# Axionis47/GAT-Recommendation

Hardware: AMD Instinct MI355X
Metric: training sessions/sec + Recall@10 parity, 82k-node graph, 1/2/4/8 MI355X (higher is better)
Workload: dtype fp32

## Files before the change

### gat-recommendation_amd/csrc/gtr_opt.hip

```cpp

#include <hipcub/hipcub.hpp>
#include <rocprim/device/device_radix_sort.hpp>

#include <cstdarg>
#include <cstdio>

#include "gtr_rows.cuh"
#include <string.h>

#include "gtr_wgrad.cuh"

namespace gtr {

static thread_local char g_err[512] = "";

void set_error(const char* fmt, ...) {
  va_list ap;
  va_start(ap, fmt);
  vsnprintf(g_err, sizeof(g_err), fmt, ap);
  va_end(ap);
}

}

// ... 693 lines not shown
      s_acc[tid] = acc;
      __syncthreads();
      if (tid == 0) {
        float t = 0.0f;
        for (int q = 0; q < GTR_BLOCK; ++q) t += s_acc[q];
        a.tl.loss_out[0] = t;
        if (a.tl.loss_acc) a.tl.loss_acc[0] += (double)t;
      }
    } else if (blk == 0 && a.tl.loss_acc && tid == 0) {
      a.tl.loss_acc[0] += (double)a.tl.loss_out[0];
    }
  }
}

struct WgradRowsK {
  WgradK w;
  gtr_batch bt;
  gtr_tail tl;
  gtr_adam opt;
  int T, nb_wg;
};

template <int D>
__global__ __launch_bounds__(GTR_TAIL_BLOCK) void k_wgrad_rows(WgradRowsK a) {
  const int blk = blockIdx.x, tid = threadIdx.x;
  if (blk < a.nb_wg) {
    if (tid >= GTR_BLOCK) return;
    wgrad_block(a.w, blk);
    return;
  }
  __shared__ AdamStep s_st;
  __shared__ int32_t s_t;
  __shared__ int s_ready;
  if (tid == 0) s_ready = 0;
  __syncthreads();
  if (tid >= GTR_BLOCK) {
    if (tid == GTR_BLOCK) {
      const int64_t t = *a.opt.step_dev + a.opt.step_offset;
      s_st.init(a.opt, t);
      s_t = (int32_t)t;
      __hip_atomic_store(&s_ready, 1, __ATOMIC_RELEASE, __HIP_MEMORY_SCOPE_WORKGROUP);
    }
    return;
  }
  auto wait = [&]() {
    while (__hip_atomic_load(&s_ready, __ATOMIC_ACQUIRE, __HIP_MEMORY_SCOPE_WORKGROUP) == 0)
      __builtin_amdgcn_s_sleep(1);
  };
  rows_body<D>((blk - a.nb_wg) * GTR_BLOCK + tid, a.bt, a.T, a.tl.skeys, a.tl.svals, a.tl.dx0, a.tl.se,
               a.tl.coef_tgt, a.tl.coef_neg, a.tl.table, a.tl.table_m, a.tl.table_v, nullptr, s_st,
               a.tl.lazy_consts ? a.tl.stamp : nullptr, s_t, wait);
}

template <int D>
__global__ __launch_bounds__(GTR_BLOCK) void k_scatter_rows(gtr_batch bt, int mode, const float* src,
                                                            const float* coef_tgt, const float* coef_neg,
                                                            float* dense) {
  constexpr int VPL = D >= 64 ? D / 64 : 1;
  const int lane = threadIdx.x & 63, wave = threadIdx.x >> 6;
  const int r = blockIdx.x * GTR_WAVES + wave;
  const int d0 = lane * VPL;
  if (d0 >= D) return;
  const int N = bt.hdr[0], B = bt.hdr[1];
  int key;
  const float* s;
  float c;
  if (mode == 0) {
    if (r >= N) return;
    key = bt.node_item[r];
    s = src + (size_t)r * D;
    c = 1.0f;
  } else {
    if (r >= B * (1 + bt.n_neg)) return;
    if (r < B) {
      key = bt.target[r];
      s = src + (size_t)r * D;
      c = coef_tgt[r];
    } else {
      const int q = r - B;
      key = bt.negatives[q];
      s = src + (size_t)(q / bt.n_neg) * D;
      c = coef_neg[q];
    }
  }
  if (key <= 0) return;
#pragma unroll
  for (int q = 0; q < VPL; ++q) atomicAdd(dense + (size_t)key * D + d0 + q, c * s[d0 + q]);
}

__global__ void k_step_end(int64_t* step_dev, uint32_t* rng_ctr, const float* loss_part, int nparts,
                           float* loss_out) {
  __shared__ float s_acc[64];
  const int tid = threadIdx.x;
  float acc = 0.0f;
  if (loss_part)
    for (int q = tid; q < nparts; q += 64) acc += loss_part[(size_t)q * 2] + loss_part[(size_t)q * 2 + 1];
  s_acc[tid] = acc;
  __syncthreads();
  if (tid == 0) {
    if (loss_part && loss_out) {
      float t = 0.0f;
      for (int q = 0; q < 64; ++q) t += s_acc[q];
      loss_out[0] = t;
    }
    if (step_dev) *step_dev += 1;
    if (rng_ctr) *rng_ctr += 1;
// ... 975 lines not shown
  k.bt = *bt;
  k.tl = t;
  k.opt = *opt;
  k.T = num_items;
  k.D = D;
  k.P = n_chunks;
  k.stride = slab_stride;
  k.cnt = tile_cnt;
  const char* wm = getenv("GTR_WGRAD");
  bool mfma = (bt->n_cap + n_chunks - 1) / n_chunks >= GTR_WGRAD_MFMA_ROWS;
  if (wm && !strcmp(wm, "mfma")) mfma = true;
  if (wm && !strcmp(wm, "valu")) mfma = false;
  if (slab_stride % 4) mfma = false;
  for (int l = 0; l < cfg->num_layers; ++l)
    if (reinterpret_cast<uintptr_t>(layer_slab[l]) % 16) mfma = false;
  int nj = 0, wblocks = 0;
  const int rc = build_wjobs(cfg, bt, layers, t.dx0, pe_tab, layer_slab, pe_slab, layer_flat, pe_flat, n_chunks, 0,
                             cfg->num_layers, k.jobs, nj, wblocks, mfma);
  if (rc) return rc;
  int tiles = 0;
  for (int i = 0; i < nj; ++i) {
    k.jobs[i].tile0 = tiles;
    tiles += k.jobs[i].nt;
    if (k.jobs[i].fW < 0 && k.jobs[i].fB < 0) { set_error("gtr_step_tail_wgrad: a job without flat offsets"); return GTR_E_ARG; }
  }
  if (tiles > tile_cnt_len) {
    set_error("gtr_step_tail_wgrad: %d tile counters needed, %d given", tiles, tile_cnt_len);
    return GTR_E_ARG;
  }
  k.njobs = nj;
  k.nb_wg = wblocks;
  k.nb_rows = (int)(((int64_t)m_cap * (D / 4) + GTR_BLOCK - 1) / GTR_BLOCK);
  int64_t tot = 0;
  for (int i = 0; i < nseg; ++i) {
    k.segs[i] = segs[i];
    tot += segs[i].len;
  }
  k.nseg = nseg;
  k.small_total = (int)tot;
  k.nb_small = (int)((tot + GTR_BLOCK - 1) / GTR_BLOCK);
  if (k.nb_small == 0 && (t.loss_part || t.loss_acc)) k.nb_small = 1;
  const int grid = k.nb_wg + k.nb_rows + k.nb_small;
  hipStream_t s = (hipStream_t)stream;
  switch (D) {
    case 32: hipLaunchKernelGGL(k_step_tail_wgrad<32>, dim3(grid), dim3(GTR_BLOCK), 0, s, k); break;
    case 64: hipLaunchKernelGGL(k_step_tail_wgrad<64>, dim3(grid), dim3(GTR_BLOCK), 0, s, k); break;
    case 128: hipLaunchKernelGGL(k_step_tail_wgrad<128>, dim3(grid), dim3(GTR_BLOCK), 0, s, k); break;
    default: hipLaunchKernelGGL(k_step_tail_wgrad<256>, dim3(grid), dim3(GTR_BLOCK), 0, s, k); break;
  }
  GTR_HIP_CHECK_LAUNCH();
  return GTR_OK;
}

static bool dp_layout_ok(const gtr_dp_layout* l, int dim) {
  return l && l->world >= 1 && l->m_cap > 0 && l->flat_total >= 0 && l->loss_off >= l->flat_total &&
         l->keys_off > l->loss_off && l->rows_off >= l->keys_off + l->m_cap && (l->rows_off & 3) == 0 &&
         l->words >= l->rows_off + (int64_t)l->m_cap * dim && (l->words & 3) == 0;
}

int gtr_dp_pack(const gtr_batch* bt, int num_items, int dim, const gtr_tail* tail, const gtr_segment* segs, int nseg,
                const gtr_dp_layout* lay, float* pack, gtr_stream_t stream) {
  if (!bt || !tail || !pack || !dim_ok(dim) || !dp_layout_ok(lay, dim) || nseg < 0 || nseg > GTR_SMALL_MAX_SEG ||
      lay->m_cap != bt->n_cap + bt->b_cap * (1 + bt->n_neg) || !tail->skeys || !tail->svals || !tail->dx0 ||
      !tail->se || !tail->coef_tgt || !tail->coef_neg || (!tail->loss_part && !tail->loss_out)) {
    set_error("gtr_dp_pack: bad arguments");
    return GTR_E_ARG;
  }
  DpPackK k{};
  k.bt = *bt;
  k.tl = *tail;
  k.lay = *lay;
  k.pack = pack;
  k.T = num_items;
  hipStream_t s = (hipStream_t)stream;
  k.windowed = lay->m_cap > GTR_BEGIN_MCAP ? 1 : 0;
  if (k.windowed) {
    if (!tail->carry) { set_error("gtr_dp_pack: large batch (m_cap > %d) needs the carry scratch", GTR_BEGIN_MCAP); return GTR_E_ARG; }
    const int nwin = (lay->m_cap + TW - 1) / TW;
    k.nb_rows = nwin;
    if (nwin > 1) {
      switch (dim) {
        case 32: hipLaunchKernelGGL(k_tail_carry<32>, dim3(carry_blocks(lay->m_cap)), dim3(GTR_BLOCK), 0, s, *bt, num_items, *tail); break;
        case 64: hipLaunchKernelGGL(k_tail_carry<64>, dim3(carry_blocks(lay->m_cap)), dim3(GTR_BLOCK), 0, s, *bt, num_items, *tail); break;
        case 128: hipLaunchKernelGGL(k_tail_carry<128>, dim3(carry_blocks(lay->m_cap)), dim3(GTR_BLOCK), 0, s, *bt, num_items, *tail); break;
        default: hipLaunchKernelGGL(k_tail_carry<256>, dim3(carry_blocks(lay->m_cap)), dim3(GTR_BLOCK), 0, s, *bt, num_items, *tail); break;
      }
      GTR_HIP_CHECK_LAUNCH();
    }
  } else {
    k.nb_rows = (int)(((int64_t)lay->m_cap * (dim / 4) + GTR_BLOCK - 1) / GTR_BLOCK);
  }
  k.nb_small = (int)((lay->flat_total + GTR_BLOCK - 1) / GTR_BLOCK);
  if (k.nb_small == 0) k.nb_small = 1;
  k.nseg = nseg;
  for (int i = 0; i < nseg; ++i) k.segs[i] = segs[i];
  const int grid = k.nb_rows + k.nb_small;
  switch (dim) {
    case 32: hipLaunchKernelGGL(k_dp_pack<32>, dim3(grid), dim3(GTR_BLOCK), 0, s, k); break;
    case 64: hipLaunchKernelGGL(k_dp_pack<64>, dim3(grid), dim3(GTR_BLOCK), 0, s, k); break;
    case 128: hipLaunchKernelGGL(k_dp_pack<128>, dim3(grid), dim3(GTR_BLOCK), 0, s, k); break;
    default: hipLaunchKernelGGL(k_dp_pack<256>, dim3(grid), dim3(GTR_BLOCK), 0, s, k); break;
  }
  GTR_HIP_CHECK_LAUNCH();
  return GTR_OK;
}

// ... 55 lines not shown
```

### gat-recommendation_amd/etpgt/backend/_lib.py

```python

from __future__ import annotations

import ctypes as C
import os

_HERE = os.path.dirname(os.path.abspath(__file__))
PKG_ROOT = os.path.dirname(os.path.dirname(_HERE))
LIB_PATH = os.environ.get("GTR_LIB", os.path.join(PKG_ROOT, "build", "libgtr_hip.so"))

P = C.c_void_p
i32 = C.c_int32
i64 = C.c_int64
f32 = C.c_float
u32 = C.c_uint32


class GtrBatch(C.Structure):
    _fields_ = [
        ("hdr", P), ("node_item", P), ("node_ptr", P), ("in_ptr", P), ("in_src", P),
        ("out_ptr", P), ("out_edge", P), ("out_dst", P), ("target", P), ("negatives", P),
        ("node_pe", P), ("grp_row", P), ("grp_edge", P),
        ("n_cap", i32), ("b_cap", i32), ("e_cap", i32), ("n_neg", i32),
    ]

# ... 94 lines not shown
        ("flat_total", i64), ("loss_off", i64), ("keys_off", i64), ("rows_off", i64), ("words", i64),
        ("m_cap", i32), ("world", i32),
    ]


class GtrShard(C.Structure):
    _fields_ = [
        ("num_items", i32), ("world", i32), ("rank", i32), ("cap", i32), ("local_rows", i32), ("dim", i32),
        ("table", P), ("m", P), ("v", P), ("stamp", P), ("consts", P), ("consts_cap", i32), ("cap_s", i32),
        ("status", P), ("opt", GtrAdam), ("node_mark", P), ("grad_stride", i64), ("small_stride", i64),
        ("pack_parts", i32), ("pad1", i32),
    ]


GTR_LOSS = {"none": 0, "bpr": 1, "listwise": 2, "sampled_softmax": 2, "dual": 3}
RO_FWD, RO_LOSS, RO_BWD = 1, 2, 4
SMALL_MAX_SEG = 48

_SIGS = {
    "gtr_version": (C.c_int, []),
    "gtr_abi_version": (C.c_int, []),
    "gtr_source_hash": (C.c_char_p, []),
    "gtr_last_error": (C.c_char_p, []),
    "gtr_device_check": (C.c_int, [C.c_int]),
    "gtr_conv_fwd": (C.c_int, [P, P, P, P, C.c_int, P]),
    "gtr_readout_loss": (C.c_int, [P, P, P, P, P, P]),
    "gtr_conv_bwd": (C.c_int, [P, P, P, C.c_int, P, P]),
    "gtr_qkvs_fwd": (C.c_int, [P, P, P, P, C.c_int, P]),
    "gtr_attn_fwd": (C.c_int, [P, P, P, C.c_int, P]),
    "gtr_attn_bwd": (C.c_int, [P, P, P, C.c_int, P]),
    "gtr_qkvs_bwd": (C.c_int, [P, P, P, C.c_int, P, P]),
    "gtr_ffn_fwd": (C.c_int, [P, P, P, C.c_int, P]),
    "gtr_ffn_bwd": (C.c_int, [P, P, P, C.c_int, P]),
    "gtr_ffn_wgrad": (C.c_int, [P, P, P, C.c_int, P, C.c_int, i64, P]),
    "gtr_wgrad": (C.c_int, [P, P, P, P, P, P, P, C.c_int, i64, C.c_int, C.c_int, P]),
    "gtr_adamw_small": (C.c_int, [P, P, P, P, i64, P, C.c_int, P, P]),
    "gtr_contrib_prep": (C.c_int, [P, C.c_int, P, P, P, P, P]),
    "gtr_contrib_sort_bytes": (C.c_int, [C.c_int, C.c_int, C.POINTER(C.c_size_t)]),
    "gtr_contrib_sort": (C.c_int, [P, P, P, P, C.c_int, C.c_int, P, C.c_size_t, P]),
    "gtr_adamw_rows": (C.c_int, [P, C.c_int, C.c_int, P, P, P, P, P, P, P, P, P, P, P, P]),
    "gtr_adamw_sweep": (C.c_int, [C.c_int, C.c_int, P, P, P, P, P, P]),
    "gtr_scatter_rows": (C.c_int, [P, C.c_int, C.c_int, P, P, P, P, P]),
    "gtr_step_end": (C.c_int, [P, P, P, C.c_int, P, P]),
    "gtr_readout_grid": (C.c_int, [C.c_int]),
    "gtr_dp_pack": (C.c_int, [P, C.c_int, C.c_int, P, P, C.c_int, P, P, P]),
    "gtr_dp_tail": (C.c_int, [P, C.c_int, C.c_int, P, P, P, P, P, P]),
    "gtr_dp_union_stamp": (C.c_int, [P, i64, C.c_int, P, P, P]),
    "gtr_step_begin": (C.c_int, [P, C.c_int, P, P, P, P, P, P, P, P, C.c_size_t, P]),
    "gtr_step_tail": (C.c_int, [P, C.c_int, C.c_int, P, P, C.c_int, P, P]),
    "gtr_step_tail_wgrad": (C.c_int, [P, P, P, P, P, P, C.c_int, C.c_int64, P, P, C.c_int, P, P, C.c_int, P, P,
                                      C.c_int, P]),
    "gtr_wgrad_rows": (C.c_int, [P, P, P, P, P, P, P, C.c_int, i64, C.c_int, C.c_int, C.c_int, P, P, P]),
    "gtr_step_tail_small": (C.c_int, [P, C.c_int, C.c_int, P, P, C.c_int, P, P]),
    "gtr_step_begin_lazy": (C.c_int, [P, C.c_int, C.c_int, P, P, P, P, P, P, P, P, C.c_size_t, P, P]),
    "gtr_lazy_flush": (C.c_int, [C.c_int, C.c_int, P, P, P, P]),
    "gtr_tail_carry_floats": (C.c_int, [C.c_int, C.c_int]),
    "gtr_edge_hash_slots": (C.c_int, [i64, C.POINTER(i64)]),
    "gtr_edge_hash_build": (C.c_int, [P, i64, P, i64, P]),
    "gtr_session_counts": (C.c_int, [P, P, i64, C.c_int, P, P, P]),
    "gtr_build_batch": (C.c_int, [P, P, i64, C.c_int, P, P, C.c_int, C.c_int, u32, P, P, P, P, P]),
    "gtr_build_batch_strided": (C.c_int, [P, P, i64, C.c_int, P, P, C.c_int, i64, C.c_int, u32, P, P, P, P, P]),
    "gtr_lap_build": (C.c_int, [P, P, C.c_int, P, P, P]),
    "gtr_lap_plan": (C.c_int, [P, C.c_int, C.c_int, P, P, P, P, P]),
    "gtr_lap_spmm": (C.c_int, [P, P, C.c_int, C.c_int, P, i64, P, i64, P, P, P, f32, f32, P]),
    "gtr_lap_gram": (C.c_int, [P, P, C.c_int, C.c_int, P, C.c_int, P, P]),
    "gtr_shard_route_scratch": (C.c_int, [C.c_int, C.c_int, C.POINTER(C.c_size_t)]),
    "gtr_shard_route": (C.c_int, [P, P, P, P, P, P, P, P, P, P, C.c_int, P, P, C.c_size_t, P]),
    "gtr_shard_serve": (C.c_int, [P, P, P, P]),
    "gtr_shard_pack": (C.c_int, [P, P, P, P, P, C.c_int, P, P, P]),
    "gtr_shard_update": (C.c_int, [P, P, P, P, P, i64, P]),
    "gtr_topk_workspace_bytes": (C.c_int, [C.c_int, C.c_int, C.c_int, C.POINTER(C.c_size_t)]),
    "gtr_score_topk": (C.c_int, [P, C.c_int, C.c_int, P, C.c_int, C.c_int, P, P, P, C.c_size_t, P]),
    "gtr_score_topk_masked": (C.c_int, [P, C.c_int, C.c_int, P, C.c_int, C.c_int, P, P, P, P, P, C.c_size_t, P]),
    "gtr_target_rank_workspace_bytes": (C.c_int, [C.c_int, C.c_int, C.POINTER(C.c_size_t)]),
    "gtr_target_rank": (C.c_int, [P, C.c_int, C.c_int, P, C.c_int, P, P, i64, P, P, P, C.c_size_t, P]),
}

EXPORTS = tuple(_SIGS)

_lib = None


class GtrLibraryMissing(RuntimeError):
    pass


def lib():
    global _lib
    if _lib is None:
        if not os.path.exists(LIB_PATH):
            raise GtrLibraryMissing(
                f"libgtr_hip.so not found at {LIB_PATH}; build it with "
                "`python -c 'import __graft_entry__ as g; g.build()'` or "
                "`make -C gat-recommendation_amd/csrc` (hipcc --offload-arch=gfx950)"
            )
        h = C.CDLL(LIB_PATH, mode=C.RTLD_GLOBAL)
        for name, (res, args) in _SIGS.items():
            fn = getattr(h, name)
            fn.restype = res
            fn.argtypes = args
        if h.gtr_abi_version() != ABI_VERSION:
            raise RuntimeError("libgtr_hip.so ABI version mismatch")
        _lib = h
    return _lib


# ... 19 lines not shown
```

### gat-recommendation_amd/etpgt/train/fused.py

```python

from __future__ import annotations

import ctypes as C
import os

import torch

from etpgt.backend import _lib as L
from etpgt.backend.engine import Engine, readout_grid
from etpgt.data.batch import Caps, SessionBatch


class FusedTrainStep:
    def __init__(self, model, lr: float = 1e-3, betas=(0.9, 0.999), eps: float = 1e-8,
                 weight_decay: float = 1e-5, decoupled: bool = True, loss: str = "bpr",
                 temperature: float = 1.0, alpha: float = 0.7, caps: Caps | None = None,
                 use_graph: bool = True, data_parallel: bool | None = None, process_group=None,
                 lazy: bool = False, sync_bn: bool = False, lagged: bool = False, shard_table: bool = False):
        if loss not in ("bpr", "listwise", "dual", "sampled_softmax"):
            raise ValueError(f"Unknown loss type: {loss}")
        if getattr(model, "use_ffn", False):
            if os.environ.get("GTR_TAILW") == "1":
                raise NotImplementedError("the FFN variant (use_ffn=True) has no GTR_TAILW step")
            if sync_bn and not (model.embedding_dim in (64, 128) and getattr(model, "ffn_expansion", 4) == 4):
# ... 180 lines not shown
        self.early_union = (self.data_parallel and chain and not self.sync_bn and not self.lagged
                            and not self.shard_table and os.environ.get("GTR_DP_EARLY", "0") == "1")
        if self.early_union:
            wts = [0.0] * eng.L + wts[eng.L:]
        slots = len(wts)
        if chain and not self.shard_table and not self.split \
                and (not self.data_parallel or self.early_union or self.lagged) \
                and self.ws.g_cap <= 128 and slots <= L.SWEEP_SLOTS:
            sw = L.GtrSweep()
            sw.table = eng.model.item_embedding.weight.data_ptr()
            sw.m, sw.v, sw.stamp = self.m_tab.data_ptr(), self.v_tab.data_ptr(), self.stamp.data_ptr()
            sw.opt = self.adam
            tot, acc = sum(wts), 0.0
            if self.early_union:
                self.keys_all = torch.zeros(self.world, m_cap, dtype=torch.int32, device=self.dev)
            for i in range(L.SWEEP_SLOTS + 1):
                sw.bounds[i] = eng.T if i >= slots else int(eng.T * acc / tot)
                if i < slots:
                    acc += wts[i]
            sw.dim = eng.D
            sw.blocks = int(os.environ.get("GTR_SWEEP_BLOCKS", 0 if eng.D <= 64 else 128))
            sw.lag = 1 if self.lagged else 0
            sw.consts = self.lazy_consts.data_ptr() if self.lagged else None
            self.sweep = sw
            self.cfg.sweep = C.addressof(sw)
            t.sweep_from = eng.T
        t.lazy_consts = self.lazy_consts.data_ptr() if self.lazy else None
        nc = int(L.lib().gtr_tail_carry_floats(m_cap, eng.D))
        self.carry = torch.zeros(max(nc, 4), dtype=torch.float32, device=self.dev) if nc > 0 else None
        t.carry = self.carry.data_ptr() if self.carry is not None else None
        self.cfg.begin, self.cfg.ctr_add, t.rng_inc = None, 0, None
        if self.begin_fused:
            bg = L.GtrBegin()
            bg.skeys, bg.svals, bg.stamp = self.skeys.data_ptr(), self.svals.data_ptr(), self.stamp.data_ptr()
            bg.step_dev, bg.num_items = self.step_dev.data_ptr(), eng.T
            self.begin_st = bg
            self.cfg.begin = C.addressof(bg)
            self.cfg.ctr_add = 1
            t.rng_inc = eng.rng_ctr.data_ptr()
        self.tail = t
        if self.shard_table:
            from etpgt.train.sharded import ShardExchange

            self.dp = None
            self.shard = ShardExchange(self, self.shard_state)
        elif self.data_parallel:
            from etpgt.train.distributed import DpExchange

            self.dp = DpExchange(self, self.group)
        if self.sync_bn:
            self._sync_alloc()
        self.tail_wgrad = (self.dp is None and self.shard is None and m_cap <= 8192
                           and (self.lazy or t.sweep_from >= eng.T) and os.environ.get("GTR_TAILW", "0") == "1")
        if self.tail_wgrad:
            self.tile_cnt = torch.zeros(4096, dtype=torch.int32, device=self.dev)
            lay = eng.flat.layout
            gb = [i for i in range(self.nseg)
                  if any(self.segs[i].begin == lay.seg(f"{l}.{n}").begin for l in range(eng.L) for n in ("gamma", "beta"))]
            self.segs_gb = (L.GtrSegment * max(1, len(gb)))()
            for j, i in enumerate(gb):
                self.segs_gb[j] = self.segs[i]
            self.nseg_gb = len(gb)
            self.layer_flat = (C.c_int64 * (3 * eng.L))(*[lay.seg(f"{l}.{n}").begin for l in range(eng.L)
                                                          for n in ("w_all", "b_all", "w_beta")])
            self.pe_flat = (C.c_int64 * 2)(lay.seg("pe.w").begin, lay.seg("pe.b").begin) if eng.K > 0 else None
        self.rows_early = (self.dp is None and self.shard is None and m_cap <= 8192 and not self.tail_wgrad
                           and os.environ.get("GTR_ROWS_EARLY", "1") != "0")
        self.graph = None
        self.graph_pe = None
        self.graph_b = None
        self.resident = None
        self.resident_graphs = None

    def workspace_ranges(self) -> list[tuple[str, int, int]]:
        out = []

        def add(name, t):
            if isinstance(t, torch.Tensor) and t.is_cuda and t.numel() > 0:
                out.append((name, t.data_ptr(), t.data_ptr() + t.numel() * t.element_size()))

        for name in ("keys", "vals", "skeys", "svals", "sort_tmp", "blob", "carry", "m_tab", "v_tab", "stamp",
                     "m_flat", "v_flat"):
            add(name, getattr(self, name, None))
        for name, t in vars(self.ws).items():
            add(f"ws.{name}", t)
        for l, lay in enumerate(getattr(self.ws, "layers", [])):
            for name, t in lay.items():
                add(f"ws.layers[{l}].{name}", t)
        return out

    def check_workspace_overlap(self) -> None:
        rs = sorted(self.workspace_ranges(), key=lambda r: r[1])
        for (n0, a0, b0), (n1, a1, b1) in zip(rs, rs[1:]):
            if a1 < b0 and not (a0 == a1 and b0 == b1):
                raise RuntimeError(f"workspace overlap: {n0} [{a0:#x}, {b0:#x}) and {n1} [{a1:#x}, {b1:#x})")

    def ensure_caps(self, batch: SessionBatch):
        N, B, E, n = batch.sizes()
        if self.data_parallel and self.world > 1:
            import torch.distributed as dist

            dev = self.dev if dist.get_backend(self.group) != "gloo" else "cpu"
            t = torch.tensor([N, B, E], dtype=torch.int64, device=dev)
            dist.all_reduce(t, op=dist.ReduceOp.MAX, group=self.group)
            N, B, E = (int(v) for v in t.tolist())
        if self.caps is None:
            self._bind(Caps.bucket(2 * N, B, 2 * E, n))
        elif not self.caps.fits(N, B, E, n):
            if n != self.caps.n_neg:
                raise ValueError("the number of negatives per session must stay fixed")
            self._bind(self.caps.grow(N, B, E, n))

    def load(self, batch: SessionBatch) -> bool:
        self.ensure_caps(batch)
        batch.check_ids(self.eng.T)
        _, host = batch.packed(self.caps)
        src = torch.from_numpy(host)
        self.blob.copy_(src.to(self.dev, non_blocking=True) if self.blob.device != src.device else src)
        if self.eng.K > 0 and batch.laplacian_pe is not None:
            pe = batch.laplacian_pe
# ... 50 lines not shown
                pa = torch.zeros(W, rows_f * (1 + 2 * D), dtype=torch.float32, device=self.dev)
                ga = torch.zeros(W, rows_b * 2 * D, dtype=torch.float32, device=self.dev)
            st.bn_part_all, st.bn_gpart_all = pa.data_ptr(), ga.data_ptr()
            st.nparts_fwd, st.nparts_bwd = W * rows_f, W * rows_b
            self.sync_bufs.append((pa, ga, rows_f * (1 + 2 * D), rows_b * 2 * D))
        self.cfg.consumer_reduce = 1
        self.cfg.sync_bn = 1
        self.cfg.split_sync = 1 if self.split else 0

    def _gather_fwd(self, l):
        from etpgt.train.distributed import all_gather_packs

        if self.sync_alias:
            return
        pa, _, n, _ = self.sync_bufs[l]
        all_gather_packs(pa, self.ws.layers[l]["bn_part"].view(-1)[:n], self.group)

    def _gather_bwd(self, l):
        from etpgt.train.distributed import all_gather_packs

        if self.sync_alias:
            return
        _, ga, _, n = self.sync_bufs[l]
        src = self.ws.layers[l]["bn_gsum" if self.split else "bn_gpart"]
        all_gather_packs(ga, src.view(-1)[:n], self.group)

    def _begin(self, bs, st):
        eng = self.eng
        lib = L.lib()
        if self.builder is not None:
            self.builder.launch(bs, self.caps, st, self._builder_B)
        if self.begin_fused:
            return
        if self.lazy:
            L.check(lib.gtr_step_begin_lazy(C.byref(bs), eng.T, eng.D, self.keys.data_ptr(), self.vals.data_ptr(),
                                            self.skeys.data_ptr(), self.svals.data_ptr(), self.stamp.data_ptr(),
                                            self.step_dev.data_ptr(), eng.rng_ctr.data_ptr(),
                                            self.sort_tmp.data_ptr(), self.sort_tmp.numel(), C.byref(self.lz), st),
                    "step_begin_lazy")
        else:
            L.check(lib.gtr_step_begin(C.byref(bs), eng.T, self.keys.data_ptr(), self.vals.data_ptr(),
                                       self.skeys.data_ptr(), self.svals.data_ptr(), self.stamp.data_ptr(),
                                       self.step_dev.data_ptr(), eng.rng_ctr.data_ptr(), self.sort_tmp.data_ptr(),
                                       self.sort_tmp.numel(), st), "step_begin")

    def _launch_a(self, with_pe: bool):
        eng = self.eng
        ws, cfg = self.ws, self.cfg
        bs = self.bs_pe if with_pe else self.bs
        st = torch.cuda.current_stream(self.dev).cuda_stream
        self._begin(bs, st)
        eng.run_forward(ws, cfg, bs, L.RO_FWD | L.RO_LOSS | L.RO_BWD, self.loss_kind, self.temperature, self.alpha,
                        split=self.split)
        eng.run_backward(ws, cfg, bs, wgrad=not self.tail_wgrad, split=self.split,
                         rows=(self.tail, self.adam) if self.rows_early else None)
        if self.dp is not None:
            self.dp.launch_pack(bs, st)

    def _launch_b(self, with_pe: bool):
        eng = self.eng
        bs = self.bs_pe if with_pe else self.bs
        st = torch.cuda.current_stream(self.dev).cuda_stream
        if self.dp is not None:
            self.dp.launch_tail(bs, st)
        elif self.tail_wgrad:
            pe = self.model.laplacian_pe._cached_pe if eng.K > 0 else None
            ws = self.ws
            L.check(L.lib().gtr_step_tail_wgrad(C.byref(self.cfg), C.byref(bs), ws.structs,
                                                None if pe is None else pe.data_ptr(), ws.slab_ptrs,
                                                None if ws.pe_slab is None else ws.pe_slab.data_ptr(), ws.P,
                                                eng.flat.layout.slab_stride, self.layer_flat, self.pe_flat, eng.T,
                                                C.byref(self.tail), self.segs_gb, self.nseg_gb, C.byref(self.adam),
                                                self.tile_cnt.data_ptr(), self.tile_cnt.numel(), st),
                    "step_tail_wgrad")
        elif self.rows_early:
            L.check(L.lib().gtr_step_tail_small(C.byref(bs), eng.T, eng.D, C.byref(self.tail), self.segs, self.nseg,
                                                C.byref(self.adam), st), "step_tail_small")
        else:
            L.check(L.lib().gtr_step_tail(C.byref(bs), eng.T, eng.D, C.byref(self.tail), self.segs, self.nseg,
                                          C.byref(self.adam), st), "step_tail")

    def _pieces(self, with_pe: bool):
        if self.shard is not None:
            self.shard.forked = False
            return self._shard_pieces(with_pe)
        if self.dp is None:
            def whole():
                self._launch_a(with_pe)
                self._launch_b(with_pe)
            return [(whole, None)]
        if not self.sync_bn and not (self.early_union and self.sweep is not None):
            return [(lambda: self._launch_a(with_pe), self.dp.exchange), (lambda: self._launch_b(with_pe), None)]
        if not self.sync_bn:
            return self._early_pieces(with_pe)
        eng, ws, cfg = self.eng, self.ws, self.cfg
        bs = self.bs_pe if with_pe else self.bs
        lib = L.lib()
        Lc = eng.L

        def st():
            return torch.cuda.current_stream(self.dev).cuda_stream

        ffn = ws.ffns is not None

        def fwd(l):
            def f():
                if l == 0:
                    self._begin(bs, st())
                if ffn and l > 0:
                    eng.ffn_fwd(ws, cfg, bs, l - 1, st())
                eng.layer_fwd(ws, cfg, bs, l, eng.fill_embed(), st(), self.split)
            return f

        def head():
            if ffn:
                eng.ffn_fwd(ws, cfg, bs, Lc - 1, st())
            eng.run_head(ws, cfg, bs, L.RO_FWD | L.RO_LOSS | L.RO_BWD, self.loss_kind, self.temperature, self.alpha)
            if ffn:
                eng.ffn_bwd(ws, cfg, bs, Lc - 1, st())

        def bwd(l):
            def f():
                eng.layer_bwd(ws, cfg, bs, l, st(), self.split)
                if ffn and l > 0:
                    eng.ffn_bwd(ws, cfg, bs, l - 1, st())
                if l == 0:
                    eng._wgrad(ws, cfg, bs, 0, Lc, st())
# ... 468 lines not shown
```

### include/gtr.h

```cpp
#ifndef GTR_H
#define GTR_H

#include <stddef.h>
#include <stdint.h>

#ifdef __cplusplus
extern "C" {
#endif

#define GTR_ABI_VERSION 9

#define GTR_OK 0
#define GTR_E_ARG 1001
#define GTR_E_DEVICE 1002

typedef void* gtr_stream_t;

typedef struct gtr_batch {
  const int32_t* hdr;
  const int32_t* node_item;
  const int32_t* node_ptr;
  const int32_t* in_ptr;
  const int32_t* in_src;
  const int32_t* out_ptr;
// ... 222 lines not shown
} gtr_lazy;

int gtr_step_begin_lazy(const gtr_batch* bt, int num_items, int dim, int32_t* keys, int32_t* vals, int32_t* skeys,
                        int32_t* svals, int32_t* stamp, int64_t* step_dev, uint32_t* rng_ctr, void* tmp,
                        size_t tmp_bytes, const gtr_lazy* lazy, gtr_stream_t stream);
int gtr_lazy_flush(int num_items, int dim, int32_t* stamp, const int64_t* step_dev, const gtr_lazy* lazy,
                   gtr_stream_t stream);

typedef struct gtr_tail {
  const int32_t* skeys;
  const int32_t* svals;
  const float* dx0;
  const float* se;
  const float* coef_tgt;
  const float* coef_neg;
  float* table;
  float* table_m;
  float* table_v;
  int32_t* stamp;
  float* flat;
  float* flat_m;
  float* flat_v;
  int64_t flat_total;
  const float* loss_part;
  float* loss_out;
  int32_t loss_nparts;
  int32_t pad0;
  float* carry;
  int64_t sweep_from;
  const float* lazy_consts;
  uint32_t* rng_inc;
  double* loss_acc;
} gtr_tail;

int gtr_tail_carry_floats(int m_cap, int dim);

int gtr_step_tail(const gtr_batch* bt, int num_items, int dim, const gtr_tail* tail,
                  const gtr_segment* segs, int nseg, const gtr_adam* opt, gtr_stream_t stream);

int gtr_step_tail_wgrad(const gtr_config* cfg, const gtr_batch* bt, const gtr_layer* layers, const float* pe_tab,
                        float* const* layer_slab, float* pe_slab, int n_chunks, int64_t slab_stride,
                        const int64_t* layer_flat, const int64_t* pe_flat, int num_items, const gtr_tail* tail,
                        const gtr_segment* segs, int nseg, const gtr_adam* opt, uint32_t* tile_cnt, int tile_cnt_len,
                        gtr_stream_t stream);

int gtr_wgrad_rows(const gtr_config* cfg, const gtr_batch* bt, const gtr_layer* layers, const float* dx0,
                   const float* pe_tab, float* const* layer_slab, float* pe_slab, int n_chunks, int64_t slab_stride,
                   int l_begin, int l_end, int num_items, const gtr_tail* tail, const gtr_adam* opt,
                   gtr_stream_t stream);

int gtr_step_tail_small(const gtr_batch* bt, int num_items, int dim, const gtr_tail* tail,
                        const gtr_segment* segs, int nseg, const gtr_adam* opt, gtr_stream_t stream);

typedef struct gtr_dp_layout {
  int64_t flat_total, loss_off, keys_off, rows_off, words;
  int32_t m_cap, world;
} gtr_dp_layout;

int gtr_dp_pack(const gtr_batch* bt, int num_items, int dim, const gtr_tail* tail, const gtr_segment* segs,
                int nseg, const gtr_dp_layout* lay, float* pack, gtr_stream_t stream);

int gtr_dp_union_stamp(const int32_t* keys_all, int64_t n, int num_items, int32_t* stamp, const int64_t* step_dev,
                       gtr_stream_t stream);

int gtr_dp_tail(const gtr_batch* bt, int num_items, int dim, const gtr_tail* tail, const gtr_dp_layout* lay,
                const float* recv, int32_t* slot, const gtr_adam* opt, gtr_stream_t stream);

typedef struct gtr_shard {
  int32_t num_items;
  int32_t world;
  int32_t rank;
  int32_t cap;
  int32_t local_rows;
  int32_t dim;
  float* table;
  float* m;
  float* v;
  int32_t* stamp;
  float* consts;
  int32_t consts_cap;
  int32_t cap_s;
  int32_t* status;
  gtr_adam opt;
  int32_t* node_mark;
  int64_t grad_stride;
  int64_t small_stride;
  int32_t pack_parts;
  int32_t pad1;
} gtr_shard;

int gtr_shard_route_scratch(int m_cap, int world, size_t* bytes);
int gtr_shard_route(const gtr_batch* bt, const int32_t* skeys, const int32_t* svals, const gtr_shard* sh,
                    int32_t* send_ids, int32_t* ckeys, int32_t* node_item_c, int32_t* target_c, int32_t* negatives_c,
                    const float* pe_tab, int pe_k, float* node_pe, void* scratch, size_t scratch_bytes,
                    gtr_stream_t stream);
int gtr_shard_serve(const gtr_shard* sh, const int32_t* recv_ids, float* send_rows, gtr_stream_t stream);
int gtr_shard_pack(const gtr_batch* bt, const gtr_shard* sh, const gtr_tail* tail, const int32_t* ckeys,
                   const gtr_segment* segs, int nseg, float* send_grads, float* small_pack, gtr_stream_t stream);
int gtr_shard_update(const gtr_shard* sh, const gtr_tail* tail, const int32_t* recv_ids, const float* recv_grads,
                     const float* small_all, int64_t small_words, gtr_stream_t stream);

int gtr_topk_workspace_bytes(int B, int num_items, int k, size_t* bytes);
int gtr_score_topk(const float* se, int B, int dim, const float* table, int num_items, int k,
                   int64_t* out_idx, float* out_score, void* ws, size_t ws_bytes, gtr_stream_t stream);
int gtr_score_topk_masked(const float* se, int B, int dim, const float* table, int num_items, int k,
                          const int32_t* excl_ptr, const int32_t* excl_ids, int64_t* out_idx, float* out_score,
// ... 50 lines not shown
```

Measured before the change: 451,200.

## Fuse weight-gradient, AdamW update and row tail into one step-end kernel

Adds a single step-end kernel for small batches. It computes the per-layer weight gradients (matmul tiles, column sums, gate terms) in LDS staging, applies AdamW to the flat parameters, and runs the embedding-row updates and the loss reduction in the same launch. The backward pass then skips its separate wgrad launches when this path is enabled, which is on by default when the batch fits. This cuts kernel launches and global round-trips of gradient slabs per step. In exchange it uses scalar VALU FMAs rather than MFMA and has fixed staging limits.

```diff
diff --git a/gat-recommendation_amd/csrc/gtr_opt.hip b/gat-recommendation_amd/csrc/gtr_opt.hip
--- a/gat-recommendation_amd/csrc/gtr_opt.hip
+++ b/gat-recommendation_amd/csrc/gtr_opt.hip
@@ -769,6 +769,351 @@
                a.tl.lazy_consts ? a.tl.stamp : nullptr, s_t, wait);
 }
 
+#define GTR_SE_ROWS 256
+#define GTR_SE_OM 2
+#define GTR_SE_ON 1
+#define GTR_SE_CW 16
+#define GTR_SE_MAXP (GTR_BLOCK / GTR_SE_CW)
+#define GTR_SE_SEGS 16
+#define GTR_SE_YOFF ((GTR_SE_ROWS + GTR_SE_MAXP) * GTR_SE_CW)
+#define GTR_SE_UOFF (2 * GTR_SE_YOFF)
+#define GTR_SE_LDS (GTR_SE_ROWS * 16 * (GTR_SE_OM + GTR_SE_ON))
+static_assert(GTR_SE_UOFF + GTR_SE_ROWS <= GTR_SE_LDS, "GATE staging must fit the MM staging buffer");
+static_assert(GTR_BLOCK <= GTR_SE_LDS, "the loss partials reuse the staging buffer");
+
+struct SEJob {
+  int type, M1, M2, lda, ldb, tn, hasb, pad0;
+  const float* A;
+  const float* B;
+  const int32_t* bidx;
+  const float* agg;
+  const float* s;
+  int64_t fW, fB;
+};
+
+struct StepEndK {
+  gtr_batch bt;
+  gtr_tail tl;
+  gtr_adam opt;
+  int T, P, D, njobs, nb_tiles, nb_rows, nb_gb, nseg;
+  int blk0s[GTR_MAX_WJOBS];
+  int gb0s[GTR_SE_SEGS];
+  SEJob jobs[GTR_MAX_WJOBS];
+  gtr_segment segs[GTR_SE_SEGS];
+};
+
+struct SEChunks {
+  int N, per, lg;
+  __device__ __forceinline__ SEChunks(const int32_t* hdr, int n_cap, int P) {
+    N = min(max(hdr[0], 0), n_cap);
+    per = (N + P - 1) / P;
+    lg = per <= 16 ? 4 : 32 - __clz(per - 1);
+  }
+  __device__ __forceinline__ int row(int slot) const {
+    const int p = slot >> lg, r = slot & ((1 << lg) - 1);
+    const int t = p * per + r;
+    return r < per && t < N ? t : -1;
+  }
+};
+
+template <int OM, int ON, class Wait>
+__device__ __forceinline__ void se_mm_tile(const SEJob& J, int tile, const int32_t* hdr, int n_cap, int P, float* S,
+                                           float* fp, float* fm, float* fv, const AdamStep& s_st, Wait wait) {
+  constexpr int TM = 16 * OM, TN = 16 * ON, LS = TM + TN;
+  constexpr int A4 = TM / 4, B4 = TN / 4;
+  constexpr int NQA = GTR_SE_ROWS * A4 / GTR_BLOCK, NQB = GTR_SE_ROWS * B4 / GTR_BLOCK;
+  static_assert(GTR_SE_ROWS * LS <= GTR_SE_LDS, "MM staging");
+  const int tid = threadIdx.x;
+  const int tm = tile / J.tn, tq = tile - tm * J.tn;
+  const int m0 = tm * TM, n0 = tq * TN;
+  const int ty = tid >> 4, tx = tid & 15;
+  const SEChunks ch(hdr, n_cap, P);
+  int64_t e[OM][ON];
+  float pv[OM][ON], mv[OM][ON], vv[OM][ON];
+#pragma unroll
+  for (int i = 0; i < OM; ++i)
+#pragma unroll
+    for (int q = 0; q < ON; ++q) {
+      const int m = m0 + ty * OM + i, n = n0 + tx * ON + q;
+      e[i][q] = -1;
+      if (m < J.M1) {
+        if (n < J.M2) e[i][q] = J.fW + (int64_t)m * J.M2 + n;
+        else if (n == J.M2 && J.hasb) e[i][q] = J.fB + m;
+      }
+      pv[i][q] = mv[i][q] = vv[i][q] = 0.0f;
+      if (e[i][q] >= 0) {
+        pv[i][q] = fp[e[i][q]];
+        mv[i][q] = fm[e[i][q]];
+        vv[i][q] = fv[e[i][q]];
+      }
+    }
+  int tb[NQB];
+#pragma unroll
+  for (int q = 0; q < NQB; ++q) {
+    const int t = ch.row((tid + q * GTR_BLOCK) / B4);
+    tb[q] = t >= 0 && J.bidx ? J.bidx[t] : t;
+  }
+  const float4 z4 = make_float4(0.f, 0.f, 0.f, 0.f);
+  float4 av[NQA], bv[NQB];
+#pragma unroll
+  for (int q = 0; q < NQA; ++q) {
+    const int idx = tid + q * GTR_BLOCK;
+    const int t = ch.row(idx / A4), col = m0 + (idx % A4) * 4;
+    av[q] = z4;
+    if (t >= 0 && col < J.M1) av[q] = *reinterpret_cast<const float4*>(J.A + (size_t)t * J.lda + col);
+  }
+#pragma unroll
+  for (int q = 0; q < NQB; ++q) {
+    const int idx = tid + q * GTR_BLOCK;
+    const int col = n0 + (idx % B4) * 4;
+    bv[q] = z4;
+    if (tb[q] >= 0) {
+      if (col < J.M2) bv[q] = *reinterpret_cast<const float4*>(J.B + (size_t)tb[q] * J.ldb + col);
+      else if (col == J.M2 && J.hasb) bv[q].x = 1.0f;
+    }
+  }
+#pragma unroll
+  for (int q = 0; q < NQA; ++q) {
+    const int idx = tid + q * GTR_BLOCK;
+    *reinterpret_cast<float4*>(S + (idx / A4) * LS + (idx % A4) * 4) = av[q];
+  }
+#pragma unroll
+  for (int q = 0; q < NQB; ++q) {
+    const int idx = tid + q * GTR_BLOCK;
+    *reinterpret_cast<float4*>(S + (idx / B4) * LS + TM + (idx % B4) * 4) = bv[q];
+  }
+  __syncthreads();
+  float g[OM][ON];
+#pragma unroll
+  for (int i = 0; i < OM; ++i)
+#pragma unroll
+    for (int q = 0; q < ON; ++q) g[i][q] = 0.0f;
+  for (int p = 0; p < P; ++p) {
+    const int t0 = p * ch.per;
+    if (t0 >= ch.N) break;
+    const int nr = min(ch.N - t0, ch.per);
+    const float* Sp = S + (p << ch.lg) * LS;
+    float acc[OM][ON];
+#pragma unroll
+    for (int i = 0; i < OM; ++i)
+#pragma unroll
+      for (int q = 0; q < ON; ++q) acc[i][q] = 0.0f;
+    for (int k0 = 0; k0 < nr; k0 += 8) {
+#pragma unroll
+      for (int k = 0; k < 8; ++k) {
+        const float* r = Sp + (k0 + k) * LS;
+        float ar[OM], br[ON];
+#pragma unroll
+        for (int i = 0; i < OM; ++i) ar[i] = r[ty * OM + i];
+#pragma unroll
+        for (int q = 0; q < ON; ++q) br[q] = r[TM + tx * ON + q];
+#pragma unroll
+        for (int i = 0; i < OM; ++i)
+#pragma unroll
+          for (int q = 0; q < ON; ++q) acc[i][q] = __builtin_fmaf(ar[i], br[q], acc[i][q]);
+      }
+    }
+#pragma unroll
+    for (int i = 0; i < OM; ++i)
+#pragma unroll
+      for (int q = 0; q < ON; ++q) g[i][q] += acc[i][q];
+  }
+  wait();
+  const AdamStep st = s_st;
+#pragma unroll
+  for (int i = 0; i < OM; ++i)
+#pragma unroll
+    for (int q = 0; q < ON; ++q) {
+      if (e[i][q] < 0) continue;
+      st.apply(pv[i][q], mv[i][q], vv[i][q], g[i][q]);
+      fp[e[i][q]] = pv[i][q];
+      fm[e[i][q]] = mv[i][q];
+      fv[e[i][q]] = vv[i][q];
+    }
+}
+
+template <class Wait>
+__device__ __forceinline__ void se_col_tile(const SEJob& J, int tile, const int32_t* hdr, int n_cap, int P, int D,
+                                            float* S, float (*cv)[GTR_SE_MAXP][GTR_SE_CW], float* fp, float* fm,
+                                            float* fv, const AdamStep& s_st, Wait wait) {
+  constexpr int CW = GTR_SE_CW, C4 = CW / 4, NQ = GTR_SE_ROWS * C4 / GTR_BLOCK;
+  static_assert(GTR_SE_ROWS == GTR_BLOCK, "one du word per thread");
+  const int tid = threadIdx.x;
+  const bool gate = J.type == WJ_GATE;
+  const int c0 = tile * CW;
+  const SEChunks ch(hdr, n_cap, P);
+  const int nown = gate ? 3 * CW : CW;
+  const int64_t e = gate ? J.fW + (int64_t)(tid / CW) * D + c0 + tid % CW : J.fB + c0 + tid % CW;
+  float pv = 0.0f, mv = 0.0f, vv = 0.0f;
+  if (tid < nown) {
+    pv = fp[e];
+    mv = fm[e];
+    vv = fv[e];
+  }
+  const float4 z4 = make_float4(0.f, 0.f, 0.f, 0.f);
+  const float* X = gate ? J.agg : J.A;
+  const int ldx = gate ? D : J.lda;
+  float4 xv[NQ], yv[NQ];
+#pragma unroll
+  for (int q = 0; q < NQ; ++q) {
+    const int idx = tid + q * GTR_BLOCK;
+    const int t = ch.row(idx / C4), col = c0 + (idx % C4) * 4;
+    xv[q] = z4;
+    yv[q] = z4;
+    if (t >= 0) {
+      xv[q] = *reinterpret_cast<const float4*>(X + (size_t)t * ldx + col);
+      if (gate) yv[q] = *reinterpret_cast<const float4*>(J.s + (size_t)t * J.lda + col);
+    }
+  }
+  float uv = 0.0f;
+  if (gate) {
+    const int t = ch.row(tid);
+    if (t >= 0) uv = J.A[t];
+  }
+#pragma unroll
+  for (int q = 0; q < NQ; ++q) {
+    const int idx = tid + q * GTR_BLOCK;
+    const int slot = idx / C4, o = (slot + (slot >> ch.lg)) * CW + (idx % C4) * 4;
+    *reinterpret_cast<float4*>(S + o) = xv[q];
+    if (gate) *reinterpret_cast<float4*>(S + GTR_SE_YOFF + o) = yv[q];
+  }
+  if (gate) S[GTR_SE_UOFF + tid] = uv;
+  __syncthreads();
+  const int c = tid % CW, p = tid / CW;
+  if (p < P) {
+    constexpr int PH = 16;
+    float s0[PH], s1[PH], s2[PH];
+#pragma unroll
+    for (int ph = 0; ph < PH; ++ph) s0[ph] = s1[ph] = s2[ph] = 0.0f;
+    const int nr = max(0, min(ch.N - p * ch.per, ch.per));
+    const float* Sx = S + ((p << ch.lg) + p) * CW + c;
+    const float* Su = S + GTR_SE_UOFF + (p << ch.lg);
+    for (int r0 = 0; r0 < nr; r0 += PH) {
+#pragma unroll
+      for (int ph = 0; ph < PH; ++ph) {
+        const float x = Sx[(r0 + ph) * CW];
+        if (gate) {
+          const float y = Sx[GTR_SE_YOFF + (r0 + ph) * CW];
+          const float u = Su[r0 + ph];
+          s0[ph] = __builtin_fmaf(u, x, s0[ph]);
+          s1[ph] = __builtin_fmaf(u, y, s1[ph]);
+          s2[ph] = __builtin_fmaf(u, x - y, s2[ph]);
+        } else {
+          s0[ph] += x;
+        }
+      }
+    }
+    float g0 = 0.0f, g1 = 0.0f, g2 = 0.0f;
+#pragma unroll
+    for (int ph = 0; ph < PH; ++ph) {
+      g0 += s0[ph];
+      g1 += s1[ph];
+      g2 += s2[ph];
+    }
+    cv[0][p][c] = g0;
+    if (gate) {
+      cv[1][p][c] = g1;
+      cv[2][p][c] = g2;
+    }
+  }
+  __syncthreads();
+  if (tid >= nown) return;
+  float g = 0.0f;
+  for (int q = 0; q < P; ++q) g += cv[tid / CW][q][tid % CW];
+  wait();
+  const AdamStep st = s_st;
+  st.apply(pv, mv, vv, g);
+  fp[e] = pv;
+  fm[e] = mv;
+  fv[e] = vv;
+}
+
+template <int D>
+__global__ __launch_bounds__(GTR_TAIL_BLOCK) void k_step_end_small(StepEndK a) {
+  __shared__ AdamStep s_st;
+  __shared__ int32_t s_t;
+  __shared__ int s_ready;
+  __shared__ __attribute__((aligned(16))) float s_x[GTR_SE_LDS];
+  __shared__ float s_cv[3][GTR_SE_MAXP][GTR_SE_CW];
+  const int blk = blockIdx.x, tid = threadIdx.x;
+  if (tid == 0) s_ready = 0;
+  __syncthreads();
+  if (tid >= GTR_BLOCK) {
+    if (tid == GTR_BLOCK) {
+      const int64_t t = *a.opt.step_dev + a.opt.step_offset;
+      s_st.init(a.opt, t);
+      s_t = (int32_t)t;
+      __hip_atomic_store(&s_ready, 1, __ATOMIC_RELEASE, __HIP_MEMORY_SCOPE_WORKGROUP);
+      if (blk == a.nb_tiles + a.nb_rows && a.tl.rng_inc) *a.tl.rng_inc += 1;
+    }
+    return;
+  }
+  auto wait = [&]() {
+    while (__hip_atomic_load(&s_ready, __ATOMIC_ACQUIRE, __HIP_MEMORY_SCOPE_WORKGROUP) == 0)
+      __builtin_amdgcn_s_sleep(1);
+  };
+  if (blk < a.nb_tiles) {
+    int jid = 0;
+#pragma unroll
+    for (int i = 1; i < GTR_MAX_WJOBS; ++i) jid += i < a.njobs && blk >= a.blk0s[i] ? 1 : 0;
+    const SEJob& J = a.jobs[jid];
+    const int tile = blk - a.blk0s[jid];
+    if (J.type == WJ_MM)
+      se_mm_tile<GTR_SE_OM, GTR_SE_ON>(J, tile, a.bt.hdr, a.bt.n_cap, a.P, s_x, a.tl.flat, a.tl.flat_m, a.tl.flat_v,
+                                       s_st, wait);
+    else
+      se_col_tile(J, tile, a.bt.hdr, a.bt.n_cap, a.P, a.D, s_x, s_cv, a.tl.flat, a.tl.flat_m, a.tl.flat_v, s_st, wait);
+    return;
+  }
+  if (blk < a.nb_tiles + a.nb_rows) {
+    rows_body<D>((blk - a.nb_tiles) * GTR_BLOCK + tid, a.bt, a.T, a.tl.skeys, a.tl.svals, a.tl.dx0, a.tl.se,
+                 a.tl.coef_tgt, a.tl.coef_neg, a.tl.table, a.tl.table_m, a.tl.table_v, nullptr, s_st,
+                 a.tl.lazy_consts ? a.tl.stamp : nullptr, s_t, wait);
+    return;
+  }
+  const int sb = blk - a.nb_tiles - a.nb_rows;
+  const bool loss = sb == 0 && a.tl.loss_part;
+  const int lnp = loss ? a.tl.loss_nparts : 0;
+  float2 lp = make_float2(0.f, 0.f);
+  if (tid < lnp) lp = make_float2(a.tl.loss_part[(size_t)tid * 2], a.tl.loss_part[(size_t)tid * 2 + 1]);
+  if (a.nseg > 0) {
+    int sg = 0;
+#pragma unroll
+    for (int i = 1; i < GTR_SE_SEGS; ++i) sg += i < a.nseg && sb >= a.gb0s[i] ? 1 : 0;
+    const gtr_segment& S = a.segs[sg];
+    const int64_t off = (int64_t)(sb - a.gb0s[sg]) * GTR_BLOCK + tid;
+    if (off < S.len) {
+      const int64_t e = S.begin + off;
+      float pv = a.tl.flat[e], mv = a.tl.flat_m[e], vv = a.tl.flat_v[e];
+      float g = 0.0f;
+      for (int q = 0; q < S.nparts; ++q) g += S.src[(int64_t)q * S.pstride + off];
+      wait();
+      const AdamStep st = s_st;
+      st.apply(pv, mv, vv, g);
+      a.tl.flat[e] = pv;
+      a.tl.flat_m[e] = mv;
+      a.tl.flat_v[e] = vv;
+    }
+  }
+  if (loss) {
+    float acc = 0.0f;
+    if (tid < lnp) acc += lp.x + lp.y;
+    for (int q = tid + GTR_BLOCK; q < lnp; q += GTR_BLOCK)
+      acc += a.tl.loss_part[(size_t)q * 2] + a.tl.loss_part[(size_t)q * 2 + 1];
+    s_x[tid] = acc;
+    __syncthreads();
+    if (tid == 0) {
+      float t = 0.0f;
+      const int nq = lnp < GTR_BLOCK ? lnp : GTR_BLOCK;
+      for (int q = 0; q < nq; ++q) t += s_x[q];
+      a.tl.loss_out[0] = t;
+      if (a.tl.loss_acc) a.tl.loss_acc[0] += (double)t;
+    }
+  } else if (sb == 0 && a.tl.loss_acc && tid == 0) {
+    a.tl.loss_acc[0] += (double)a.tl.loss_out[0];
+  }
+}
+
 template <int D>
 __global__ __launch_bounds__(GTR_BLOCK) void k_scatter_rows(gtr_batch bt, int mode, const float* src,
                                                             const float* coef_tgt, const float* coef_neg,
@@ -1850,6 +2195,120 @@
   return GTR_OK;
 }
 
+static int step_end_slots(int n_cap, int n_chunks) {
+  const int per = (n_cap + n_chunks - 1) / n_chunks;
+  int pad = 16;
+  while (pad < per) pad *= 2;
+  return n_chunks * pad;
+}
+
+int gtr_step_end_small_fits(int n_cap, int n_chunks, int pe_k) {
+  return n_cap > 0 && n_chunks > 0 && n_chunks <= GTR_SE_MAXP && step_end_slots(n_cap, n_chunks) <= GTR_SE_ROWS &&
+                 pe_k >= 0 && pe_k % 4 == 0
+             ? 1
+             : 0;
+}
+
+int gtr_step_end_small(const gtr_config* cfg, const gtr_batch* bt, const gtr_layer* layers, const float* pe_tab,
+                       int n_chunks, const int64_t* layer_flat, const int64_t* pe_flat, int num_items,
+                       const gtr_tail* tail, const gtr_segment* segs, int nseg, const gtr_adam* opt,
+                       gtr_stream_t stream) {
+  if (!cfg || !bt || !layers || !layer_flat || !tail || !opt || !opt->step_dev || num_items <= 0 || nseg < 0 ||
+      nseg > GTR_SE_SEGS || (nseg > 0 && !segs) || !dim_ok(cfg->dim) || n_chunks <= 0 || !bt->hdr ||
+      3 * cfg->num_layers + 1 > GTR_MAX_WJOBS || (cfg->pe_k > 0 && !pe_flat)) {
+    set_error("gtr_step_end_small: bad arguments");
+    return GTR_E_ARG;
+  }
+  const gtr_tail& t = *tail;
+  const int D = cfg->dim;
+  const int m_cap = bt->n_cap + bt->b_cap * (1 + bt->n_neg);
+  if (m_cap > GTR_BEGIN_MCAP || !gtr_step_end_small_fits(bt->n_cap, n_chunks, cfg->pe_k)) {
+    set_error("gtr_step_end_small: batch too large (n_cap %d in %d chunks, m_cap %d, pe_k %d; one staging round holds "
+              "%d row slots): use gtr_wgrad_rows + gtr_step_tail_small",
+              bt->n_cap, n_chunks, m_cap, cfg->pe_k, GTR_SE_ROWS);
+    return GTR_E_ARG;
+  }
+  if (!t.lazy_consts && t.sweep_from < num_items) {
+    set_error("gtr_step_end_small: the untouched-row sweep must run in the chain (sweep_from == num_items)");
+    return GTR_E_ARG;
+  }
+  if (!t.skeys || !t.svals || !t.dx0 || !t.se || !t.coef_tgt || !t.coef_neg || !t.table || !t.table_m ||
+      !t.table_v || !t.stamp || !t.flat || !t.flat_m || !t.flat_v || t.flat_total <= 0 ||
+      (t.loss_part && (!t.loss_out || t.loss_nparts < 0))) {
+    set_error("gtr_step_end_small: missing buffers");
+    return GTR_E_ARG;
+  }
+  StepEndK k{};
+  k.bt = *bt;
+  k.tl = t;
+  k.opt = *opt;
+  k.T = num_items;
+  k.P = n_chunks;
+  k.D = D;
+  WJob wj[GTR_MAX_WJOBS];
+  int nj = 0, unused = 0;
+  if (const int rc = build_wjobs(cfg, bt, layers, t.dx0, pe_tab, nullptr, nullptr, layer_flat, pe_flat, 1, 0,
+                                 cfg->num_layers, wj, nj, unused, false))
+    return rc;
+  constexpr int TM = 16 * GTR_SE_OM, TN = 16 * GTR_SE_ON;
+  auto al16 = [](const void* p) { return reinterpret_cast<uintptr_t>(p) % 16 == 0; };
+  int blocks = 0;
+  for (int i = 0; i < nj; ++i) {
+    const WJob& w = wj[i];
+    SEJob& j = k.jobs[i];
+    j = SEJob{};
+    j.type = w.type; j.M1 = w.M1; j.M2 = w.M2; j.lda = w.lda; j.ldb = w.ldb;
+    j.A = w.A; j.B = w.B; j.bidx = w.bidx; j.agg = w.agg; j.s = w.s; j.fW = w.fW; j.fB = w.fB;
+    k.blk0s[i] = blocks;
+    bool ok;
+    if (w.type == WJ_MM) {
+      j.hasb = w.tn * 64 > w.M2 ? 1 : 0;
+      j.tn = (w.M2 + j.hasb + TN - 1) / TN;
+      blocks += ((w.M1 + TM - 1) / TM) * j.tn;
+      ok = w.A && w.B && al16(w.A) && al16(w.B) && w.lda % 4 == 0 && w.ldb % 4 == 0 && w.M1 % 4 == 0 &&
+           w.M2 % 4 == 0 && w.fW >= 0 && w.fW + (int64_t)w.M1 * w.M2 <= t.flat_total &&
+           (!j.hasb || (w.fB >= 0 && w.fB + w.M1 <= t.flat_total));
+    } else if (w.type == WJ_COLSUM) {
+      blocks += w.M1 / GTR_SE_CW;
+      ok = w.A && al16(w.A) && w.lda % 4 == 0 && w.M1 % GTR_SE_CW == 0 && w.fB >= 0 && w.fB + w.M1 <= t.flat_total;
+    } else {
+      blocks += D / GTR_SE_CW;
+      ok = w.A && w.agg && w.s && al16(w.agg) && al16(w.s) && w.lda % 4 == 0 && w.fW >= 0 &&
+           w.fW + 3 * (int64_t)D <= t.flat_total;
+    }
+    if (!ok) {
+      set_error("gtr_step_end_small: job %d: a null or misaligned (16 B) operand, or flat offsets outside the buffer", i);
+      return GTR_E_ARG;
+    }
+  }
+  k.njobs = nj;
+  k.nb_tiles = blocks;
+  k.nb_rows = (int)(((int64_t)m_cap * (D / 4) + GTR_BLOCK - 1) / GTR_BLOCK);
+  int gb = 0;
+  for (int i = 0; i < nseg; ++i) {
+    const gtr_segment& s = segs[i];
+    if (s.begin < 0 || s.len < 0 || s.begin + s.len > t.flat_total || !s.src || s.nparts < 0) {
+      set_error("gtr_step_end_small: segment %d outside the flat buffer", i);
+      return GTR_E_ARG;
+    }
+    k.segs[i] = s;
+    k.gb0s[i] = gb;
+    gb += (int)((s.len + GTR_BLOCK - 1) / GTR_BLOCK);
+  }
+  k.nseg = nseg;
+  k.nb_gb = gb > 0 ? gb : 1;
+  const int grid = k.nb_tiles + k.nb_rows + k.nb_gb;
+  hipStream_t s = (hipStream_t)stream;
+  switch (D) {
+    case 32: hipLaunchKernelGGL(k_step_end_small<32>, dim3(grid), dim3(GTR_TAIL_BLOCK), 0, s, k); break;
+    case 64: hipLaunchKernelGGL(k_step_end_small<64>, dim3(grid), dim3(GTR_TAIL_BLOCK), 0, s, k); break;
+    case 128: hipLaunchKernelGGL(k_step_end_small<128>, dim3(grid), dim3(GTR_TAIL_BLOCK), 0, s, k); break;
+    default: hipLaunchKernelGGL(k_step_end_small<256>, dim3(grid), dim3(GTR_TAIL_BLOCK), 0, s, k); break;
+  }
+  GTR_HIP_CHECK_LAUNCH();
+  return GTR_OK;
+}
+
 static bool dp_layout_ok(const gtr_dp_layout* l, int dim) {
   return l && l->world >= 1 && l->m_cap > 0 && l->flat_total >= 0 && l->loss_off >= l->flat_total &&
          l->keys_off > l->loss_off && l->rows_off >= l->keys_off + l->m_cap && (l->rows_off & 3) == 0 &&
diff --git a/gat-recommendation_amd/etpgt/backend/_lib.py b/gat-recommendation_amd/etpgt/backend/_lib.py
--- a/gat-recommendation_amd/etpgt/backend/_lib.py
+++ b/gat-recommendation_amd/etpgt/backend/_lib.py
@@ -170,6 +170,8 @@
                                       C.c_int, P]),
     "gtr_wgrad_rows": (C.c_int, [P, P, P, P, P, P, P, C.c_int, i64, C.c_int, C.c_int, C.c_int, P, P, P]),
     "gtr_step_tail_small": (C.c_int, [P, C.c_int, C.c_int, P, P, C.c_int, P, P]),
+    "gtr_step_end_small": (C.c_int, [P, P, P, P, C.c_int, P, P, C.c_int, P, P, C.c_int, P, P]),
+    "gtr_step_end_small_fits": (C.c_int, [C.c_int, C.c_int, C.c_int]),
     "gtr_step_begin_lazy": (C.c_int, [P, C.c_int, C.c_int, P, P, P, P, P, P, P, P, C.c_size_t, P, P]),
     "gtr_lazy_flush": (C.c_int, [C.c_int, C.c_int, P, P, P, P]),
     "gtr_tail_carry_floats": (C.c_int, [C.c_int, C.c_int]),
diff --git a/gat-recommendation_amd/etpgt/train/fused.py b/gat-recommendation_amd/etpgt/train/fused.py
--- a/gat-recommendation_amd/etpgt/train/fused.py
+++ b/gat-recommendation_amd/etpgt/train/fused.py
@@ -256,8 +256,15 @@
             self._sync_alloc()
         self.tail_wgrad = (self.dp is None and self.shard is None and m_cap <= 8192
                            and (self.lazy or t.sweep_from >= eng.T) and os.environ.get("GTR_TAILW", "0") == "1")
-        if self.tail_wgrad:
-            self.tile_cnt = torch.zeros(4096, dtype=torch.int32, device=self.dev)
+        self.rows_early = (self.dp is None and self.shard is None and m_cap <= 8192 and not self.tail_wgrad
+                           and os.environ.get("GTR_ROWS_EARLY", "1") != "0")
+        valu = os.environ.get("GTR_WGRAD") != "mfma" and -(-self.caps.n_cap // self.ws.P) < 128
+        self.step_end = (self.rows_early and self.ws.ffns is None and (self.lazy or t.sweep_from >= eng.T) and valu
+                         and bool(L.lib().gtr_step_end_small_fits(self.caps.n_cap, self.ws.P, eng.K))
+                         and os.environ.get("GTR_STEP_END", "1") != "0")
+        if self.tail_wgrad or self.step_end:
+            if self.tail_wgrad:
+                self.tile_cnt = torch.zeros(4096, dtype=torch.int32, device=self.dev)
             lay = eng.flat.layout
             gb = [i for i in range(self.nseg)
                   if any(self.segs[i].begin == lay.seg(f"{l}.{n}").begin for l in range(eng.L) for n in ("gamma", "beta"))]
@@ -268,8 +275,6 @@
             self.layer_flat = (C.c_int64 * (3 * eng.L))(*[lay.seg(f"{l}.{n}").begin for l in range(eng.L)
                                                           for n in ("w_all", "b_all", "w_beta")])
             self.pe_flat = (C.c_int64 * 2)(lay.seg("pe.w").begin, lay.seg("pe.b").begin) if eng.K > 0 else None
-        self.rows_early = (self.dp is None and self.shard is None and m_cap <= 8192 and not self.tail_wgrad
-                           and os.environ.get("GTR_ROWS_EARLY", "1") != "0")
         self.graph = None
         self.graph_pe = None
         self.graph_b = None
@@ -426,7 +431,7 @@
         self._begin(bs, st)
         eng.run_forward(ws, cfg, bs, L.RO_FWD | L.RO_LOSS | L.RO_BWD, self.loss_kind, self.temperature, self.alpha,
                         split=self.split)
-        eng.run_backward(ws, cfg, bs, wgrad=not self.tail_wgrad, split=self.split,
+        eng.run_backward(ws, cfg, bs, wgrad=not (self.tail_wgrad or self.step_end), split=self.split,
                          rows=(self.tail, self.adam) if self.rows_early else None)
         if self.dp is not None:
             self.dp.launch_pack(bs, st)
@@ -447,6 +452,12 @@
                                                 C.byref(self.tail), self.segs_gb, self.nseg_gb, C.byref(self.adam),
                                                 self.tile_cnt.data_ptr(), self.tile_cnt.numel(), st),
                     "step_tail_wgrad")
+        elif self.step_end:
+            pe = self.model.laplacian_pe._cached_pe if eng.K > 0 else None
+            L.check(L.lib().gtr_step_end_small(C.byref(self.cfg), C.byref(bs), self.ws.structs,
+                                               None if pe is None else pe.data_ptr(), self.ws.P, self.layer_flat,
+                                               self.pe_flat, eng.T, C.byref(self.tail), self.segs_gb, self.nseg_gb,
+                                               C.byref(self.adam), st), "step_end_small")
         elif self.rows_early:
             L.check(L.lib().gtr_step_tail_small(C.byref(bs), eng.T, eng.D, C.byref(self.tail), self.segs, self.nseg,
                                                 C.byref(self.adam), st), "step_tail_small")
diff --git a/include/gtr.h b/include/gtr.h
--- a/include/gtr.h
+++ b/include/gtr.h
@@ -298,6 +298,12 @@
 int gtr_step_tail_small(const gtr_batch* bt, int num_items, int dim, const gtr_tail* tail,
                         const gtr_segment* segs, int nseg, const gtr_adam* opt, gtr_stream_t stream);
 
+int gtr_step_end_small(const gtr_config* cfg, const gtr_batch* bt, const gtr_layer* layers, const float* pe_tab,
+                       int n_chunks, const int64_t* layer_flat, const int64_t* pe_flat, int num_items,
+                       const gtr_tail* tail, const gtr_segment* segs, int nseg, const gtr_adam* opt,
+                       gtr_stream_t stream);
+int gtr_step_end_small_fits(int n_cap, int n_chunks, int pe_k);
+
 typedef struct gtr_dp_layout {
   int64_t flat_total, loss_off, keys_off, rows_off, words;
   int32_t m_cap, world;
```

New measurement: 481,700 (median of 6 runs). 1.07x the previous value.
